# jh-jeong/ContraD

Hardware: AMD Instinct MI355X
Metric: discriminator-step images/sec (ContraD, SimCLR aug) (higher is better)
Workload: dtype f32; 1 GPU; SNDCGAN + ContraD D-step, CIFAR-10 32x32, global batch 512, simclr aug, nonsat loss, Adam(2e-4,(0.5,0.999)), random-init weights; global_batch=512, per_gpu_batch=512, parallelism=dp1, losses_finite=True, launch=hipGraph replay, rccl_ranks=1

## Files before the change

### contrad_amd/csrc/common.h

```cpp
#pragma once
#include <hip/hip_runtime.h>
#include <stdint.h>

#define CONTRAD_WAVE 64

#define CONTRAD_CHECK_LAUNCH()                       \
  do {                                               \
    hipError_t e__ = hipGetLastError();              \
    if (e__ != hipSuccess) return (int)e__;          \
  } while (0)

#define CONTRAD_ARG(cond)                            \
  do {                                               \
    if (!(cond)) return -22;            \
  } while (0)

#include <stdlib.h>
#ifdef CONTRAD_DEV_SWITCHES
static inline const char* contrad_dev_env(const char* name) { return getenv(name); }
#else
static inline const char* contrad_dev_env(const char*) { return nullptr; }
#endif
static inline bool contrad_dev_on(const char* name) { const char* e = contrad_dev_env(name); return !(e && e[0] == '0'); }
static inline bool contrad_dev_off_by_default(const char* name) { const char* e = contrad_dev_env(name); return e && e[0] == '1'; }
static inline int contrad_dev_int(const char* name, int dflt) { const char* e = contrad_dev_env(name); return e ? atoi(e) : dflt; }
static inline long long contrad_dev_ll(const char* name, long long dflt) { const char* e = contrad_dev_env(name); return e ? atoll(e) : dflt; }

typedef float f32x16 __attribute__((ext_vector_type(16)));
typedef float f32x4 __attribute__((ext_vector_type(4)));

static inline int cdiv(int a, int b) { return (a + b - 1) / b; }
__device__ __forceinline__ int cdiv_dev(int a, int b) { return (a + b - 1) / b; }
static inline long long cdivll(long long a, long long b) { return (a + b - 1) / b; }

__device__ __forceinline__ int xcd_remap(int b, int nb) {
  const int xcd = b & 7;
  const int q = nb >> 3, r = nb & 7;
  const int base = (xcd < r) ? xcd * (q + 1) : r * (q + 1) + (xcd - r) * q;
  return base + (b >> 3);
}

__device__ __forceinline__ float wave_sum(float v) {
#pragma unroll
  for (int o = 32; o > 0; o >>= 1) v += __shfl_xor(v, o, 64);
  return v;
}
__device__ __forceinline__ float wave_max(float v) {
#pragma unroll
  for (int o = 32; o > 0; o >>= 1) v = fmaxf(v, __shfl_xor(v, o, 64));
  return v;
}

__device__ __forceinline__ float block_sum(float v, float* red) {
  v = wave_sum(v);
  const int lane = threadIdx.x & 63, w = threadIdx.x >> 6, nw = (blockDim.x + 63) >> 6;
  __syncthreads();
  if (lane == 0) red[w] = v;
  __syncthreads();
  float t = 0.f;
  for (int i = 0; i < nw; ++i) t += red[i];
  return t;
}
```

### contrad_amd/csrc/conv_small.hip

```cpp
#include "common.h"
#include "../../include/contrad_hip.h"

namespace {

#ifndef RGB_MIN_WAVES
#define RGB_MIN_WAVES 3
#endif
typedef float f32x2 __attribute__((ext_vector_type(2)));
__device__ __forceinline__ f32x2 pk_fma(f32x2 a, f32x2 b, f32x2 c) { return __builtin_elementwise_fma(a, b, c); }

constexpr int MAX_TAPS = 9;
constexpr int MAX_CIN = 4;

struct RgbArgs {
  const float* img;
  const float* wp;
  const float* bias;
  float* y;
  int N, Cin, H, W, K, ldy, ldw, k, pad, TH;
  float in_scale, in_shift, slope, gain;
};

__device__ __forceinline__ void stage_halo(float* lds, const RgbArgs& a, int n, int h0) {
  const int HW = a.W + 2 * a.pad, HH = a.TH + 2 * a.pad;
// ... 186 lines not shown
  const long long total = (long long)a.N * a.H * a.W;
  for (long long pix0 = (long long)blockIdx.x * slots; pix0 < total; pix0 += (long long)gridDim.x * slots) {
    const long long pix = pix0 + slot;
    const bool live = pix < total;
    const long long pp = live ? pix : 0;
    const int wq = (int)(pp % a.W);
    const int h = (int)((pp / a.W) % a.H);
    const int n = (int)(pp / ((long long)a.W * a.H));
    float acc[MAX_CIN] = {0.f, 0.f, 0.f, 0.f};
    float4 md[CH];
#pragma unroll
    for (int q = 0; q < CH; ++q)
      md[q] = a.mod ? *reinterpret_cast<const float4*>(a.mod + (size_t)n * a.K + (q * tpp + cg) * 4)
                    : make_float4(1.f, 1.f, 1.f, 1.f);
#pragma unroll
    for (int kh = 0; kh < KSZ; ++kh) {
      const int ho = h + a.pad - kh;
#pragma unroll
      for (int kw = 0; kw < KSZ; ++kw) {
        const int wo = wq + a.pad - kw;
        const bool ok = live && (unsigned)ho < (unsigned)a.H && (unsigned)wo < (unsigned)a.W;
        const float m = ok ? 1.f : 0.f;
#pragma unroll
        for (int q = 0; q < CH; ++q) {
          const float4 g = *reinterpret_cast<const float4*>(
              a.gy + (ok ? ((size_t)(n * a.H + ho) * a.W + wo) * a.ldy + (q * tpp + cg) * 4 : 0));
#pragma unroll
          for (int c = 0; c < MAX_CIN; ++c) {
            const float4 ww = w[q][(kh * KSZ + kw) * MAX_CIN + c];
            acc[c] += m * (g.x * md[q].x * ww.x + g.y * md[q].y * ww.y + g.z * md[q].z * ww.z + g.w * md[q].w * ww.w);
          }
        }
      }
    }
#pragma unroll
    for (int c = 0; c < MAX_CIN; ++c)
      for (int o = tpp >> 1; o > 0; o >>= 1) acc[c] += __shfl_xor(acc[c], o, 64);
    if (live && cg < a.C) {
      float v = (cg == 0) ? acc[0] : (cg == 1) ? acc[1] : (cg == 2) ? acc[2] : acc[3];
      v += a.bias ? a.bias[cg] : 0.f;
      const size_t o = ((size_t)(n * a.C + cg) * a.H + h) * a.W + wq;
      if (a.residual) v += a.residual[o];
      if (a.act == 1) v = tanhf(v);
      a.out[o] = v * a.out_scale + a.out_shift;
    }
  }
}

constexpr int DG_CK = 32;
constexpr int DG_PS = DG_CK + 4;
__global__ __launch_bounds__(256) void rgb_dgrad3_tile_kernel(const float* __restrict__ gy, const float* __restrict__ wp,
                                                              const float* __restrict__ bias, float* __restrict__ out,
                                                              int N, int C, int H, int W, int K, int ldy, int ldw, int TH,
                                                              int act, float out_scale, float out_shift) {
  extern __shared__ __attribute__((aligned(16))) float tile[];
  const int tiles_h = cdiv_dev(H, TH);
  const int n = blockIdx.x / tiles_h, h0 = (blockIdx.x % tiles_h) * TH;
  const int HW2 = W + 2, HH2 = TH + 2;
  float* wl = tile + (size_t)HH2 * HW2 * DG_PS;
  const int r = threadIdx.x / W, c = threadIdx.x - r * W;
  const bool live = threadIdx.x < TH * W && h0 + r < H;
  float acc[3] = {0.f, 0.f, 0.f};
  for (int k0 = 0; k0 < K; k0 += DG_CK) {
    __syncthreads();
    for (int e = threadIdx.x; e < HH2 * HW2 * (DG_CK / 4); e += blockDim.x) {
      const int q = e % (DG_CK / 4), p = e / (DG_CK / 4);
      const int pr = p / HW2, pc = p - pr * HW2;
      const int h = h0 - 1 + pr, w = pc - 1;
      float4 v = make_float4(0.f, 0.f, 0.f, 0.f);
      if ((unsigned)h < (unsigned)H && (unsigned)w < (unsigned)W)
        v = *reinterpret_cast<const float4*>(gy + ((size_t)(n * H + h) * W + w) * ldy + k0 + q * 4);
      *reinterpret_cast<float4*>(tile + (size_t)p * DG_PS + q * 4) = v;
    }
    for (int e = threadIdx.x; e < 9 * 3 * (DG_CK / 4); e += blockDim.x) {
      const int q = e % (DG_CK / 4), tc = e / (DG_CK / 4);
      const int tap = tc / 3, cc = tc - tap * 3;
      float4 v = make_float4(0.f, 0.f, 0.f, 0.f);
      if (cc < C) v = *reinterpret_cast<const float4*>(wp + (size_t)(tap * C + cc) * ldw + k0 + q * 4);
      *reinterpret_cast<float4*>(wl + tc * DG_CK + q * 4) = v;
    }
    __syncthreads();
    if (live) {
#pragma unroll
      for (int kh = 0; kh < 3; ++kh)
#pragma unroll
        for (int kw = 0; kw < 3; ++kw) {
          const float4* g4 = reinterpret_cast<const float4*>(tile + (size_t)((r + 2 - kh) * HW2 + (c + 2 - kw)) * DG_PS);
          const float4* w4 = reinterpret_cast<const float4*>(wl + (kh * 3 + kw) * 3 * DG_CK);
#pragma unroll
          for (int q = 0; q < DG_CK / 4; ++q) {
            const float4 g = g4[q];
#pragma unroll
            for (int cc = 0; cc < 3; ++cc) {
              const float4 ww = w4[cc * (DG_CK / 4) + q];
              acc[cc] = fmaf(g.x, ww.x, fmaf(g.y, ww.y, fmaf(g.z, ww.z, fmaf(g.w, ww.w, acc[cc]))));
            }
          }
        }
    }
  }
  if (live) {
#pragma unroll
    for (int cc = 0; cc < 3; ++cc) {
      if (cc < C) {
        float v = acc[cc] + (bias ? bias[cc] : 0.f);
        if (act == 1) v = tanhf(v);
        out[((size_t)(n * C + cc) * H + h0 + r) * W + c] = v * out_scale + out_shift;
      }
    }
  }
}

int rgb_common_check(int N, int Cin, int H, int W, int K, int k, int ldy, int ldw) {
  CONTRAD_ARG(N > 0 && H > 0 && W > 0 && Cin == 3);
  CONTRAD_ARG(k == 1 || k == 3);
  CONTRAD_ARG(K >= 4 && (K & 3) == 0 && K <= 1024 && (1024 % K) == 0);
  CONTRAD_ARG(ldy >= K && (ldy & 3) == 0 && (ldw & 3) == 0 && ldw >= K);
  return 0;
}

int pick_th(int W) { int th = 1024 / W; return th < 1 ? 1 : (th > 32 ? 32 : th); }

}

extern "C" int contrad_rgb_conv_fwd(const float* img, const float* wp, const float* bias, float* y, int N,
                                    int Cin, int H, int W, int K, int k, int ldy, int ldw, float in_scale,
                                    float in_shift, float slope, float gain, contrad_stream_t stream) {
  int rc = rgb_common_check(N, Cin, H, W, K, k, ldy, ldw);
  if (rc) return rc;
  CONTRAD_ARG(img && wp && y);
  RgbArgs a{};
  a.img = img; a.wp = wp; a.bias = bias; a.y = y;
  a.N = N; a.Cin = Cin; a.H = H; a.W = W; a.K = K; a.ldy = ldy; a.ldw = ldw; a.k = k; a.pad = k / 2;
  a.TH = pick_th(W);
  a.in_scale = in_scale; a.in_shift = in_shift; a.slope = slope; a.gain = gain;
  const int tiles = N * cdiv(H, a.TH);
  const int grid = tiles < 4096 ? tiles : 4096;
  const size_t smem = (size_t)Cin * (a.TH + 2 * a.pad) * (W + 2 * a.pad) * sizeof(float);
  CONTRAD_ARG(smem <= 64 * 1024);
  if (k == 3) hipLaunchKernelGGL((rgb_conv_fwd_kernel<3, 3>), dim3(grid), dim3(256), smem, (hipStream_t)stream, a);
  else hipLaunchKernelGGL((rgb_conv_fwd_kernel<1, 3>), dim3(grid), dim3(256), smem, (hipStream_t)stream, a);
  CONTRAD_CHECK_LAUNCH();
  return 0;
}

static int rgb_wgrad_grid(int N, int H, int W, int k) {
  const int tiles = N * cdiv(H, pick_th(W));
  const int cap = (k == 3) ? 768 : 2048;
  return tiles < cap ? tiles : cap;
}

extern "C" long long contrad_rgb_conv_wgrad_workspace_bytes(int N, int Cin, int H, int W, int K, int k) {
  return (long long)rgb_wgrad_grid(N, H, W, k) * (k * k * Cin + 1) * K * (long long)sizeof(float);
}

extern "C" int contrad_rgb_conv_wgrad(const float* img, const float* gy, float* dwp, float* dbias, int N,
                                      int Cin, int H, int W, int K, int k, int ldy, int ldw, float in_scale,
                                      float in_shift, float* workspace, long long workspace_bytes,
                                      contrad_stream_t stream) {
  int rc = rgb_common_check(N, Cin, H, W, K, k, ldy, ldw);
  if (rc) return rc;
  CONTRAD_ARG(img && gy && dwp && workspace);
  CONTRAD_ARG(workspace_bytes >= contrad_rgb_conv_wgrad_workspace_bytes(N, Cin, H, W, K, k));
  RgbWgradArgs a{};
  a.img = img; a.gy = gy; a.partial = workspace;
  a.N = N; a.Cin = Cin; a.H = H; a.W = W; a.K = K; a.ldy = ldy; a.k = k; a.pad = k / 2; a.TH = pick_th(W);
  a.in_scale = in_scale; a.in_shift = in_shift;
  const int grid = rgb_wgrad_grid(N, H, W, k);
  size_t smem = (size_t)Cin * (a.TH + 2 * a.pad) * (W + 2 * a.pad) * sizeof(float);
  const size_t red = 256 * sizeof(float4);
  if (smem < red) smem = red;
  CONTRAD_ARG(smem <= 64 * 1024);
  if (k == 3) hipLaunchKernelGGL((rgb_conv_wgrad_kernel<3, 3>), dim3(grid), dim3(256), smem, (hipStream_t)stream, a);
  else hipLaunchKernelGGL((rgb_conv_wgrad_kernel<1, 3>), dim3(grid), dim3(256), smem, (hipStream_t)stream, a);
  CONTRAD_CHECK_LAUNCH();
  const int rows = k * k * Cin;
  hipLaunchKernelGGL(rgb_wgrad_reduce_kernel, dim3(cdiv((rows + 1) * K, 16)), dim3(256), 0,
                     (hipStream_t)stream, workspace, grid, rows, K, dwp, ldw, dbias);
  CONTRAD_CHECK_LAUNCH();
  return 0;
}

extern "C" int contrad_rgb_conv_dgrad(const float* gy, const float* wp, const float* bias, const float* mod,
                                      const float* residual, float* out, int N, int C, int H, int W, int K,
                                      int k, int ldy, int ldw, int act, float out_scale, float out_shift,
                                      contrad_stream_t stream) {
  CONTRAD_ARG(gy && wp && out && N > 0 && H > 0 && W > 0 && C >= 1 && C <= MAX_CIN);
  CONTRAD_ARG((k == 1 || k == 3) && K >= 16 && K <= 512 && (K & (K - 1)) == 0 && ldy >= K && (ldy & 3) == 0);
  CONTRAD_ARG(K <= 256 || k == 1);
  CONTRAD_ARG(ldw >= K && (ldw & 3) == 0 && (act == 0 || act == 1));
  RgbDgradArgs a{};
  a.gy = gy; a.wp = wp; a.bias = bias; a.out = out; a.mod = mod; a.residual = residual;
  a.N = N; a.C = C; a.H = H; a.W = W; a.K = K; a.ldy = ldy; a.ldw = ldw; a.k = k; a.pad = k / 2;
  a.act = act; a.out_scale = out_scale; a.out_shift = out_shift;
  const long long total = (long long)N * H * W;
  if (k == 3 && !mod && !residual && C <= 3 && (K % DG_CK) == 0 && W <= 256) {
    const int TH = 256 / W < 1 ? 1 : (256 / W > H ? H : 256 / W);
    const size_t smem = ((size_t)(TH + 2) * (W + 2) * DG_PS + 9 * 3 * DG_CK) * sizeof(float);
    if (smem <= 64 * 1024) {
      hipLaunchKernelGGL(rgb_dgrad3_tile_kernel, dim3(N * cdiv(H, TH)), dim3(256), smem, (hipStream_t)stream, gy, wp, bias,
                         out, N, C, H, W, K, ldy, ldw, TH, act, out_scale, out_shift);
      CONTRAD_CHECK_LAUNCH();
      return 0;
    }
  }
  const int ch = (K > 256) ? 2 : 1;
  const int slots = 256 / (K / (4 * ch));
  long long grid = (total + slots - 1) / slots;
  if (grid > 4096) grid = 4096;
  if (k == 3) hipLaunchKernelGGL((rgb_conv_dgrad_kernel<3, 1>), dim3((int)grid), dim3(256), 0, (hipStream_t)stream, a);
  else if (ch == 1) hipLaunchKernelGGL((rgb_conv_dgrad_kernel<1, 1>), dim3((int)grid), dim3(256), 0, (hipStream_t)stream, a);
  else hipLaunchKernelGGL((rgb_conv_dgrad_kernel<1, 2>), dim3((int)grid), dim3(256), 0, (hipStream_t)stream, a);
  CONTRAD_CHECK_LAUNCH();
  return 0;
}
```

### contrad_amd/csrc/elementwise.hip

```cpp
#include "common.h"
#include "../../include/contrad_hip.h"

namespace {

constexpr int COLS_PER_THREAD = 8;

template <bool SQ>
__global__ __launch_bounds__(256) void colstats_partial_kernel(const float* __restrict__ x, long long M, int K,
                                                               int ld, int rows_per_block,
                                                               float* __restrict__ partial) {
  __shared__ float red[4][64 * COLS_PER_THREAD + 1];
  __shared__ float red2[4][64 * COLS_PER_THREAD + 1];
  const int tx = threadIdx.x & 63, ty = threadIdx.x >> 6;
  const int cbase = blockIdx.y * 64 * COLS_PER_THREAD;
  const long long r0 = (long long)blockIdx.x * rows_per_block;
  const long long r1 = (r0 + rows_per_block < M) ? r0 + rows_per_block : M;
  float s[COLS_PER_THREAD], q[COLS_PER_THREAD];
#pragma unroll
  for (int j = 0; j < COLS_PER_THREAD; ++j) { s[j] = 0.f; q[j] = 0.f; }
  for (long long r = r0 + ty; r < r1; r += 4) {
    const float* row = x + r * ld;
#pragma unroll
    for (int j = 0; j < COLS_PER_THREAD; ++j) {
      const int c = cbase + tx + 64 * j;
// ... 53 lines not shown
  __syncthreads();
  const int nstat = SQ ? 2 : 1;
  if (rr == 0 && cok) {
    float4 t = red[0][cq];
    for (int g = 1; g < RPP; ++g) { const float4 u = red[g][cq]; t.x += u.x; t.y += u.y; t.z += u.z; t.w += u.w; }
    *reinterpret_cast<float4*>(partial + ((size_t)blockIdx.x * nstat + 0) * K + c) = t;
    if (SQ) {
      float4 t2 = red2[0][cq];
      for (int g = 1; g < RPP; ++g) { const float4 u = red2[g][cq]; t2.x += u.x; t2.y += u.y; t2.z += u.z; t2.w += u.w; }
      *reinterpret_cast<float4*>(partial + ((size_t)blockIdx.x * nstat + 1) * K + c) = t2;
    }
  }
}

constexpr int CSR_E = 16, CSR_P = 16;
__global__ __launch_bounds__(256) void colstats_reduce_kernel(const float* __restrict__ partial, int nblocks,
                                                              int nstat, int K, float* __restrict__ out,
                                                              int accumulate) {
  __shared__ float red[CSR_P][CSR_E + 1];
  const int ex = threadIdx.x % CSR_E, py = threadIdx.x / CSR_E;
  const int e = blockIdx.x * CSR_E + ex;
  const int E = nstat * K;
  float s0 = 0.f, s1 = 0.f, s2 = 0.f, s3 = 0.f;
  if (e < E) {
    int b = py;
    for (; b + 3 * CSR_P < nblocks; b += 4 * CSR_P) {
      s0 += partial[(size_t)b * E + e];
      s1 += partial[(size_t)(b + CSR_P) * E + e];
      s2 += partial[(size_t)(b + 2 * CSR_P) * E + e];
      s3 += partial[(size_t)(b + 3 * CSR_P) * E + e];
    }
    for (; b < nblocks; b += CSR_P) s0 += partial[(size_t)b * E + e];
  }
  red[py][ex] = (s0 + s1) + (s2 + s3);
  __syncthreads();
  if (py == 0 && e < E) {
    float s = 0.f;
#pragma unroll
    for (int r = 0; r < CSR_P; ++r) s += red[r][ex];
    out[e] = accumulate ? out[e] + s : s;
  }
}

__global__ void bn_relu_apply_kernel(const float* __restrict__ x, float* __restrict__ y, long long M, int K,
                                     int ldx, int ldy, const float* __restrict__ stats, float count,
                                     const float* __restrict__ gamma, const float* __restrict__ beta,
                                     float eps, int perm_hw) {
  const long long total = M * K;
  const float inv_n = 1.f / count;
  for (long long e = (long long)blockIdx.x * blockDim.x + threadIdx.x; e < total;
       e += (long long)gridDim.x * blockDim.x) {
    const long long r = e / K;
    const int c = (int)(e - r * K);
    const float mean = stats[c] * inv_n;
    const float var = fmaxf(stats[K + c] * inv_n - mean * mean, 0.f);
    const float v = (x[r * ldx + c] - mean) * rsqrtf(var + eps) * gamma[c] + beta[c];
    const float o = v > 0.f ? v : 0.f;
    if (perm_hw > 1) {
      const int ch = c / perm_hw, hw = c - ch * perm_hw;
      y[r * ldy + (size_t)hw * (K / perm_hw) + ch] = o;
    } else {
      y[r * ldy + c] = o;
    }
  }
}

__global__ __launch_bounds__(256) void bn_relu_bwd_stats_kernel(const float* __restrict__ dy,
                                                                const float* __restrict__ x, long long M, int K,
                                                                int ld, const float* __restrict__ stats, float count,
                                                                const float* __restrict__ gamma,
                                                                const float* __restrict__ beta, float eps,
                                                                int rows_per_block, float* __restrict__ partial) {
  __shared__ float red[4][64 * COLS_PER_THREAD + 1];
  __shared__ float red2[4][64 * COLS_PER_THREAD + 1];
  const int tx = threadIdx.x & 63, ty = threadIdx.x >> 6;
  const int cbase = blockIdx.y * 64 * COLS_PER_THREAD;
  const long long r0 = (long long)blockIdx.x * rows_per_block;
  const long long r1 = (r0 + rows_per_block < M) ? r0 + rows_per_block : M;
  float s[COLS_PER_THREAD], q[COLS_PER_THREAD], mu[COLS_PER_THREAD], rs[COLS_PER_THREAD], ga[COLS_PER_THREAD],
      be[COLS_PER_THREAD];
#pragma unroll
  for (int j = 0; j < COLS_PER_THREAD; ++j) {
    s[j] = 0.f; q[j] = 0.f;
    const int c = cbase + tx + 64 * j;
    if (c < K) {
      mu[j] = stats[c] / count;
      rs[j] = rsqrtf(fmaxf(stats[K + c] / count - mu[j] * mu[j], 0.f) + eps);
      ga[j] = gamma[c]; be[j] = beta[c];
    } else { mu[j] = 0.f; rs[j] = 0.f; ga[j] = 0.f; be[j] = 0.f; }
  }
  for (long long r = r0 + ty; r < r1; r += 4) {
#pragma unroll
    for (int j = 0; j < COLS_PER_THREAD; ++j) {
      const int c = cbase + tx + 64 * j;
      if (c < K) {
        const float xh = (x[r * ld + c] - mu[j]) * rs[j];
        const float g = (xh * ga[j] + be[j] > 0.f) ? dy[r * ld + c] : 0.f;
        s[j] += g;
        q[j] = fmaf(g, xh, q[j]);
      }
    }
  }
#pragma unroll
  for (int j = 0; j < COLS_PER_THREAD; ++j) { red[ty][tx + 64 * j] = s[j]; red2[ty][tx + 64 * j] = q[j]; }
  __syncthreads();
  for (int e = threadIdx.x; e < 64 * COLS_PER_THREAD; e += blockDim.x) {
    const int c = cbase + e;
    if (c < K) {
      partial[((size_t)blockIdx.x * 2 + 0) * K + c] = red[0][e] + red[1][e] + red[2][e] + red[3][e];
      partial[((size_t)blockIdx.x * 2 + 1) * K + c] = red2[0][e] + red2[1][e] + red2[2][e] + red2[3][e];
// ... 368 lines not shown
```

### contrad_amd/csrc/igemm.hip

```cpp
#include "common.h"
#include <stdlib.h>
#include <string.h>
#include <algorithm>
#include <utility>
#include "../../include/contrad_hip.h"

namespace {

enum { MODE_FWD = 0, MODE_DGRAD = 1, MODE_WGRAD = 2 };
#ifndef IGEMM_BK
#define IGEMM_BK 16
#endif
constexpr int BK = IGEMM_BK;
#ifndef IGEMM_MIN_WAVES
#define IGEMM_MIN_WAVES 4
#endif
constexpr int NTHREADS = 256;

struct IgemmArgs {
  const float* A;
  const float* B;
  float* C;
  const float* bias;
  const float* addend;
// ... 856 lines not shown
  if (g_plan_override.splits > 0) want = g_plan_override.splits;
  if (want < 1) want = 1;
  long long pps = cdivll(ptiles, want);
  if (pps < 4) pps = 4;
  if (pps > ptiles) pps = ptiles;
  p.tps = (int)pps;
  p.splits = (int)cdivll(ptiles, pps);
  if (d->K <= 32 && p.bm == 128 && vec_ok(d, MODE_WGRAD) && lean_ok(d, MODE_WGRAD, pps)) p.bn = 32;
  return p;
}

__global__ __launch_bounds__(256) void fwd_k1_kernel(const float* __restrict__ x, const float* __restrict__ w, long long M,
                                                     int C, int ldx, int ldw, const float* __restrict__ bias, float slope,
                                                     float gain, float* __restrict__ y, int ldy,
                                                     const float* __restrict__ addend) {
  const int lane = threadIdx.x & 63;
  const long long m = (long long)blockIdx.x * 4 + (threadIdx.x >> 6);
  if (m >= M) return;
  const float* xr = x + m * ldx;
  float acc = 0.f;
  for (int c = lane; c < C; c += 64) acc += xr[c] * w[(long long)c * ldw];
#pragma unroll
  for (int o = 32; o >= 1; o >>= 1) acc += __shfl_xor(acc, o, 64);
  if (lane == 0) {
    float v = acc + (bias ? bias[0] : 0.f);
    v = (v > 0.f) ? v : v * slope;
    v *= gain;
    if (addend) v += addend[m * ldy];
    y[m * ldy] = v;
  }
}

__global__ void fwd_reduce_kernel(const float* __restrict__ ws, int splits, long long M, int Ncol,
                                  const float* __restrict__ bias, float slope, float gain, float* __restrict__ y,
                                  int ldy, const float* __restrict__ addend) {
  const long long total = M * Ncol;
  for (long long e = (long long)blockIdx.x * blockDim.x + threadIdx.x; e < total;
       e += (long long)gridDim.x * blockDim.x) {
    float v = 0.f;
    for (int k = 0; k < splits; ++k) v += ws[(long long)k * total + e];
    const long long m = e / Ncol;
    const int c = (int)(e - m * Ncol);
    if (bias) v += bias[c];
    v = (v > 0.f) ? v : v * slope;
    v *= gain;
    if (addend) v += addend[m * ldy + c];
    y[m * ldy + c] = v;
  }
}

void split_plan(long long M, int Ncol, int t_total, double flops, FwdPlan* p) {
  static const int cand[4][2] = {{128, 128}, {64, 128}, {128, 64}, {64, 64}};
  static const double rate[4] = {135e12, 128e12, 128e12, 115e12};
  static const int sp[8] = {1, 2, 3, 4, 6, 8, 12, 16};
  if (g_plan_override.bm > 0) {
    const int s_ = std::max(1, g_plan_override.splits);
    p->bm = g_plan_override.bm; p->bn = g_plan_override.bn;
    p->tps = cdiv(t_total, s_);
    p->splits = cdiv(t_total, p->tps);
    return;
  }
  double best = 1e30;
  for (int i = (Ncol > 64 ? 0 : 2); i < 4; ++i)
    for (int j = 0; j < 8; ++j) {
      const int s_ = sp[j];
      const int tps = cdiv(t_total, s_);
      if (s_ > 1 && tps < 8) break;
      const int splits = cdiv(t_total, tps);
      const long long tm = cdivll(M, cand[i][0]), tn = cdivll(Ncol, cand[i][1]);
      const double blocks = (double)(tm * tn) * splits;
      const double waste = (double)(tm * cand[i][0]) * (double)(tn * cand[i][1]) / ((double)M * Ncol);
      const double fill = blocks >= 768.0 ? 1.0 : blocks / 768.0;
      double t = flops * waste / (rate[i] * fill);
      if (splits > 1) t += (2.0 * splits + 1.0) * (double)M * Ncol * 4.0 / 4e12 + 4e-6;
      if (t < best) { best = t; p->bm = cand[i][0]; p->bn = cand[i][1]; p->splits = splits; p->tps = tps; }
    }
}

bool fwd_k1_ok(const contrad_conv_desc* d) {
  return d->K == 1 && d->KH == 1 && d->KW == 1 && d->H == 1 && d->W == 1 && d->stride == 1 && d->pad == 0;
}

bool splitk_enabled() {
  static const bool on = contrad_dev_on("CONTRAD_IGEMM_SPLITK");
  return on;
}

constexpr double PIXMAJOR_MAX_VALID = 0.80;
constexpr double PIXMAJOR_WGRAD_MAX_VALID = 0.85;

bool pixmajor_enabled() {
  static const bool on = contrad_dev_on("CONTRAD_PIXMAJOR");
  return on;
}

double fwd_valid_tap_fraction(const contrad_conv_desc* d) {
  long long vh = 0, vw = 0;
  for (int ho = 0; ho < d->Ho; ++ho)
    for (int kh = 0; kh < d->KH; ++kh) vh += (unsigned)(ho * d->stride - d->pad + kh) < (unsigned)d->H;
  for (int wo = 0; wo < d->Wo; ++wo)
    for (int kw = 0; kw < d->KW; ++kw) vw += (unsigned)(wo * d->stride - d->pad + kw) < (unsigned)d->W;
  return (double)(vh * vw) / ((double)d->Ho * d->Wo * d->KH * d->KW);
}

constexpr double BORDER_MAX_VALID = 0.96;
bool border_classes_ok(const contrad_conv_desc* d, int mode, int bm);
bool fwd_pixmajor_ok(const contrad_conv_desc* d, int bm);
bool dgrad_pixmajor_ok(const contrad_conv_desc* d, int bm);
bool fwd_border_ok(const contrad_conv_desc* d, int bm, double valid) {
  return valid <= BORDER_MAX_VALID && !fwd_pixmajor_ok(d, bm) && border_classes_ok(d, MODE_FWD, bm);
}
bool dgrad_border_ok(const contrad_conv_desc* d, int bm, double valid) {
  return valid <= BORDER_MAX_VALID && !dgrad_pixmajor_ok(d, bm) && border_classes_ok(d, MODE_DGRAD, bm);
}

bool fwd_pixmajor_ok(const contrad_conv_desc* d, int bm) {
  if (!pixmajor_enabled() || d->Ho * d->Wo > 256 || d->N < bm) return false;
  if ((long long)bm * d->H * d->W * d->ldx * 4 >= (1ll << 30)) return false;
  if ((long long)bm * d->Ho * d->Wo * d->ldy * 4 >= (1ll << 31)) return false;
  return fwd_valid_tap_fraction(d) <= PIXMAJOR_MAX_VALID;
}

double dgrad_valid_tap_fraction(const contrad_conv_desc* d) {
  const int s = d->stride;
  long long valid = 0, all = 0;
  for (int h = 0; h < d->H; ++h) {
// ... 835 lines not shown
```

### contrad_amd/models/gan/sndcgan.py

```python
import contextlib

import torch
import torch.nn as nn
import torch.distributed as dist

from ... import ops
from ...hostio import upload
from ... import autograd_ops as A
from .base import BaseDiscriminator, SNParams, TinyHead, _Act, make_projection

_D_CONVS = [(3, 64, 3, 1, 1), (64, 128, 4, 2, 1), (128, 128, 3, 1, 1), (128, 256, 4, 2, 1),
            (256, 256, 3, 1, 1), (256, 512, 4, 2, 1), (512, 512, 3, 1, 1)]
_SLOPE = 0.1


def _flat_views(total_sizes, device):
    offs, tot = [], 0
    for n in total_sizes:
        offs.append(tot)
        tot += ops.round_up(n, 4)
    buf = torch.empty(max(tot, 4), device=device, dtype=torch.float32)
    return buf, [buf[o:o + n] for o, n in zip(offs, total_sizes)]


# ... 380 lines not shown
            layers.append(_WB((ci, co, k, k), co))
            if j < 3:
                layers += [BNParams(co), _Act(0.0)]
            else:
                layers.append(_Act(1.0))
        self.main = nn.Sequential(*layers)
        self.sync_bn = True
        self._packed = None
        self._packed_key = None
        self._packed_filters = {}

    def sample_latent(self, n_samples):
        _device = next(self.parameters()).device
        return upload(torch.empty(n_samples, self.nz).uniform_(-1, 1), _device)

    def invalidate_cache(self):
        self._packed, self._packed_key, self._packed_filters = None, None, {}

    def _weights(self):
        ws = [self.linear.weight] + [self.main[3 * j].weight for j in range(4)]
        key = tuple((w.data_ptr(), w._version) for w in ws)
        if self._packed_key != key:
            dev = ws[0].device
            specs = [ops.SnSpec(w, fixed_scale=1.0) for w in ws]
            sizes = [s.K * s.C * s.T for s in specs]
            buf, v = _flat_views(sizes, dev)
            wps = [v[i].view(s.T * s.C, s.K) for i, s in enumerate(specs)]
            ldws = [s.K for s in specs]
            offs, scr_n = ops.sn_scratch_floats(specs)
            scratch = torch.empty(scr_n, device=dev, dtype=torch.float32)
            sigma = torch.empty(len(specs), device=dev, dtype=torch.float32)
            ops.sn_weight_prep(specs, wps, ldws, False, scratch, offs, sigma)
            self._packed, self._packed_key, self._packed_buf = wps, key, buf
            self._packed_filters = {}
        return self._packed

    def _filters(self, N):
        if not ops.FILTER_PREP:
            return None
        pf = self._packed_filters.get(N)
        if pf is None:
            reqs, H, W = [], self.s_hb, self.s_wb
            for j in range(3):
                ci, co, k, s, p = self._CONVT[j]
                H, W = 2 * H, 2 * W
                reqs.append((1, ops.dgrad_desc((N, H, W, co), self._packed[1 + j], ci, k, k, s, p), self._packed[1 + j]))
            pf = self._packed_filters[N] = ops.filter_prep(reqs, self._packed[0].device)
        return pf

    def _bn(self, x2d, bn, conv_bias, out2d, perm_hw=1):
        if not self.training:
            mean = bn.running_mean if conv_bias is None else bn.running_mean - conv_bias
            stats = torch.stack([mean, bn.running_var + mean * mean]).contiguous()
            ops.bn_relu_apply(x2d, out2d, stats, 1.0, bn.weight, bn.bias, bn.eps, perm_hw)
            return
        count = float(x2d.shape[0])
        if ops.BN_FUSED and not _sync_on(self.sync_bn):
            stats = ops.bn_batch_stats(x2d, conv_bias, bn.momentum, bn.running_mean, bn.running_var, bn.num_batches_tracked)
            ops.bn_relu_apply(x2d, out2d, stats, count, bn.weight, bn.bias, bn.eps, perm_hw)
            return
        stats = ops.colstats(x2d, with_sq=True)
        if _sync_on(self.sync_bn):
            dist.all_reduce(stats)
            count *= dist.get_world_size()
        if self.training:
            ops.bn_running_update(stats, count, conv_bias, bn.momentum, bn.running_mean, bn.running_var,
                                  bn.num_batches_tracked)
        ops.bn_relu_apply(x2d, out2d, stats, count, bn.weight, bn.bias, bn.eps, perm_hw)

    def _forward_with_grad(self, z):
        N = z.shape[0]
        hb, wb = self.s_hb, self.s_wb
        f = 512 * hb * wb
        entries = [(f, self.nz, 1, 1.0, 0, 0)]
        groups = [(self.nz, f)]
        ws = [self.linear.weight]
        for j, (ci, co, k, s, p) in enumerate(self._CONVT):
            groups.append((k * k * co, ci))
            entries.append((ci, co, k * k, 1.0, j + 1, 0))
            ws.append(self.main[3 * j].weight)
        wp = A.PackWeightsFn.apply(A.PackMeta(entries, groups), *ws)
        z = z.contiguous().float()
        h0 = A.ConvBiasActFn.apply(z.view(N, 1, 1, self.nz), wp[0], self.linear.bias, (f, 1, 1, 1, 0), 1.0, 1.0)
        y0 = _BNReLUFn.apply(h0.view(N, f), self.norm_init.weight, self.norm_init.bias, self.norm_init, None,
                             self.sync_bn)
        x = y0.view(N, 512, hb, wb).permute(0, 2, 3, 1).contiguous()
        for j in range(3):
            ci, co, k, s, p = self._CONVT[j]
            H, W = x.shape[1], x.shape[2]
            y = A.ConvDgradFn.apply(x, wp[1 + j], (N, 2 * H, 2 * W, co), (ci, k, k, s, p))
            bn = self.main[3 * j + 1]
            y2 = _BNReLUFn.apply(y.view(-1, co), bn.weight, bn.bias, bn, self.main[3 * j].bias, self.sync_bn)
            x = y2.view(N, 2 * H, 2 * W, co)
        lin = A.RgbDgradFn.apply(x, wp[4], 3, (3, 1.0))
        return 0.5 * torch.tanh(lin + self.main[9].bias.view(1, 3, 1, 1)) + 0.5

    def forward(self, z):
        if not z.is_cuda:
            raise RuntimeError('contrad_amd.G_SNDCGAN runs on the MI355X HIP path only (no CPU fallback)')
        if torch.is_grad_enabled() and any(p.requires_grad for p in self.parameters()):
            if not self.training:
                raise NotImplementedError('eval-mode BatchNorm (running statistics) is not on the training path')
            return self._forward_with_grad(z)
        wps = self._weights()
        N = z.shape[0]
        filters = self._filters(N)
        hb, wb = self.s_hb, self.s_wb
        f = 512 * hb * wb
        z = z.contiguous().float()
        h0 = ops.conv2d_fwd(z.view(N, 1, 1, self.nz), wps[0], self.linear.bias, f, 1, 1, 1, 0).view(N, f)
        x = torch.empty((N, hb, wb, 512), device=z.device, dtype=torch.float32)
        self._bn(h0, self.norm_init, None, x.view(N, f), perm_hw=hb * wb)
        for j in range(3):
            ci, co, k, s, p = self._CONVT[j]
            H, W = x.shape[1], x.shape[2]
            y = ops.conv2d_dgrad(x, wps[1 + j], (N, 2 * H, 2 * W, co), k, k, s, p, filters=filters)
            y2 = ops.as_rows(y)
            self._bn(y2, self.main[3 * j + 1], self.main[3 * j].bias, y2)
            x = y
        return ops.rgb_conv_dgrad(x, wps[4], self.main[9].bias, 3, 3, act=1, out_scale=0.5, out_shift=0.5)
```

### contrad_amd/ops.py

```python
import ctypes
import math
import os

import torch

from ._lib import ConvDesc, ContrastProblem, FilterBatch, FilterJob, FILTER_MAX_JOBS, L2normProblem, lib


def _p(t):
    return ctypes.c_void_p(t.data_ptr()) if t is not None else ctypes.c_void_p(0)


_raw_stream = getattr(torch._C, '_cuda_getCurrentRawStream', None)


def _stream_handle():
    if _raw_stream is not None:
        return _raw_stream(torch.cuda.current_device())
    return torch.cuda.current_stream().cuda_stream


def _stream():
    return ctypes.c_void_p(_stream_handle())

# ... 453 lines not shown
        b.n = len(chunk)
        for j, s in enumerate(chunk):
            i = start + j
            L = b.layers[j]
            L.w = s.w.data_ptr()
            L.u = s.u.data_ptr() if s.u is not None else None
            L.v = s.v.data_ptr() if s.v is not None else None
            L.u_snap = u_snaps[i].data_ptr() if (u_snaps is not None and u_snaps[i] is not None) else None
            L.v_snap = v_snaps[i].data_ptr() if (v_snaps is not None and v_snaps[i] is not None) else None
            L.wp = wps[i].data_ptr()
            L.gwp = gwps[i].data_ptr() if gwps is not None else None
            L.gw = gws[i].data_ptr() if gws is not None else None
            L.K, L.C, L.T, L.ldw = s.K, s.C, s.T, ldws[i]
            L.fixed_scale = s.fixed_scale
            b.scratch_off[j] = offs[i]
        yield b, start


def sn_weight_prep(specs, wps, ldws, training, scratch, offs, sigma, u_snaps=None, v_snaps=None, eps=1e-12):
    for b, start in _sn_batches(specs, wps, ldws, offs, u_snaps, v_snaps):
        lib().call('contrad_sn_weight_prep', ctypes.byref(b), int(bool(training)), float(eps), _p(scratch),
                   ctypes.c_void_p(sigma.data_ptr() + 4 * start), _stream())


def sn_weight_grad(specs, wps, ldws, gwps, gws, scratch, offs, sigma, u_snaps=None, v_snaps=None):
    for b, start in _sn_batches(specs, wps, ldws, offs, u_snaps, v_snaps, gwps, gws):
        lib().call('contrad_sn_weight_grad', ctypes.byref(b), _p(scratch),
                   ctypes.c_void_p(sigma.data_ptr() + 4 * start), _stream())


def rgb_conv_fwd(img, wp, bias, K, k, in_scale, in_shift, slope, gain, out=None):
    _chk(img, 'img'); _chk(wp, 'wp'); _chk(bias, 'bias')
    if not img.is_contiguous():
        raise RuntimeError('contrad_hip: image batch must be contiguous NCHW')
    N, Cin, H, W = img.shape
    if out is None:
        out = torch.empty((N, H, W, K), device=img.device, dtype=torch.float32)
    lib().call('contrad_rgb_conv_fwd', _p(img), _p(wp), _p(bias), _p(out), N, Cin, H, W, K, k, _ld(out),
               wp.stride(0), float(in_scale), float(in_shift), float(slope), float(gain), _stream())
    return out


def rgb_conv_wgrad(img, gy, k, in_scale, in_shift, dwp, dbias=None):
    _chk(img, 'img'); _chk(gy, 'gy'); _chk(dwp, 'dwp')
    N, Cin, H, W = img.shape
    K = gy.shape[3]
    nbytes = lib().raw('contrad_rgb_conv_wgrad_workspace_bytes')(N, Cin, H, W, K, k)
    ws = _workspace(nbytes, img.device)
    lib().call('contrad_rgb_conv_wgrad', _p(img), _p(gy), _p(dwp), _p(dbias), N, Cin, H, W, K, k, _ld(gy),
               dwp.stride(0), float(in_scale), float(in_shift), _p(ws), ctypes.c_longlong(ws.numel() * 4), _stream())
    return dwp


def rgb_conv_dgrad(gy, wp, bias, C, k, act=0, out_scale=1.0, out_shift=0.0, out=None, mod=None, residual=None):
    _chk(gy, 'gy'); _chk(wp, 'wp'); _chk(bias, 'bias'); _chk(mod, 'mod'); _chk(residual, 'residual')
    N, H, W, K = gy.shape
    if out is None:
        out = torch.empty((N, C, H, W), device=gy.device, dtype=torch.float32)
    if mod is not None and (tuple(mod.shape) != (N, K) or not mod.is_contiguous()):
        raise RuntimeError('contrad_hip: mod must be a contiguous (N, K) tensor')
    if residual is not None and (tuple(residual.shape) != (N, C, H, W) or not residual.is_contiguous()):
        raise RuntimeError('contrad_hip: residual must be a contiguous (N, C, H, W) tensor')
    lib().call('contrad_rgb_conv_dgrad', _p(gy), _p(wp), _p(bias), _p(mod), _p(residual), _p(out), N, C, H, W, K, k,
               _ld(gy), wp.stride(0), int(act), float(out_scale), float(out_shift), _stream())
    return out


def colstats(x2d, with_sq=False, out=None, accumulate=False):
    _chk(x2d, 'x')
    M, K = x2d.shape
    ld = _ld(x2d)
    if out is None:
        out = torch.empty((2 if with_sq else 1, K), device=x2d.device, dtype=torch.float32)
    nbytes = lib().raw('contrad_colstats_workspace_bytes')(ctypes.c_longlong(M), K, int(with_sq))
    ws = _workspace(nbytes, x2d.device)
    lib().call('contrad_colstats', _p(x2d), ctypes.c_longlong(M), K, ld, int(with_sq), _p(out), int(accumulate),
               _p(ws), ctypes.c_longlong(ws.numel() * 4), _stream())
    return out


def as_rows(t):
    N, H, W, C = t.shape
    return t.as_strided((N * H * W, C), (_ld(t), 1), t.storage_offset())


def bn_relu_apply(x2d, y2d, stats, count, gamma, beta, eps=1e-5, perm_hw=1):
    M, K = x2d.shape
    lib().call('contrad_bn_relu_apply', _p(x2d), _p(y2d), ctypes.c_longlong(M), K, _ld(x2d), _ld(y2d), _p(stats),
               float(count), _p(gamma), _p(beta), float(eps), int(perm_hw), _stream())
    return y2d


def bn_running_update(stats, count, conv_bias, momentum, running_mean, running_var, num_batches_tracked=None):
    K = running_mean.numel()
    if num_batches_tracked is not None and (num_batches_tracked.dtype != torch.int64 or not num_batches_tracked.is_cuda):
        raise RuntimeError('contrad_hip: num_batches_tracked must be an int64 tensor on the device')
    lib().call('contrad_bn_running_update', _p(stats), float(count), K, _p(conv_bias), float(momentum),
               _p(running_mean), _p(running_var), _p(num_batches_tracked), _stream())


def bn_batch_stats(x2d, conv_bias, momentum, running_mean, running_var, num_batches_tracked=None):
    _chk(x2d, 'x')
    M, K = x2d.shape
    if num_batches_tracked is not None and (num_batches_tracked.dtype != torch.int64 or not num_batches_tracked.is_cuda):
        raise RuntimeError('contrad_hip: num_batches_tracked must be an int64 tensor on the device')
    out = torch.empty((2, K), device=x2d.device, dtype=torch.float32)
    nbytes = lib().raw('contrad_colstats_workspace_bytes')(ctypes.c_longlong(M), K, 1)
    ws = _workspace(nbytes, x2d.device)
    lib().call('contrad_bn_batch_stats', _p(x2d), ctypes.c_longlong(M), K, _ld(x2d), _p(out), _p(conv_bias),
               float(momentum), _p(running_mean), _p(running_var), _p(num_batches_tracked), _p(ws),
               ctypes.c_longlong(ws.numel() * 4), _stream())
# ... 885 lines not shown
```

### include/contrad_hip.h

```cpp
#ifndef CONTRAD_HIP_H
#define CONTRAD_HIP_H

#ifdef __cplusplus
extern "C" {
#endif

typedef void* contrad_stream_t;

int contrad_abi_version(void);

typedef struct {
  int N, H, W, C;
  int ldx;
  int Ho, Wo, K;
  int ldy;
  int KH, KW;
  int stride, pad;
  int ldw;
} contrad_conv_desc;

int contrad_conv2d_fwd(const contrad_conv_desc* d, const float* x, const float* wp, const float* bias,
                       float* y, float slope, float gain, float* workspace, long long workspace_bytes,
                       contrad_stream_t stream);
int contrad_conv2d_fwd_add(const contrad_conv_desc* d, const float* x, const float* wp, const float* bias,
// ... 80 lines not shown
} contrad_contrast_problem;
int contrad_contrast_fwd_batched(const contrad_contrast_problem* p, int n, contrad_stream_t stream);
int contrad_contrast_bwd_batched(const contrad_contrast_problem* p, int n, contrad_stream_t stream);
typedef struct {
  const float* u;
  float* z;
  float* inv_norm;
  const float* dz;
  float* du;
  int ldu, R, D;
  int accumulate;
  int zero_rows;
} contrad_l2norm_problem;
int contrad_l2norm_fwd_batched(const contrad_l2norm_problem* p, int n, float eps, contrad_stream_t stream);
int contrad_l2norm_bwd_batched(const contrad_l2norm_problem* p, int n, contrad_stream_t stream);

#define CONTRAD_SN_MAX_LAYERS 24
#define CONTRAD_SN_MAX_PARTIALS 256
typedef struct {
  const float* w;
  float* u;
  float* v;
  float* u_snap;
  float* v_snap;
  float* wp;
  const float* gwp;
  float* gw;
  int K, C, T, ldw;
  float fixed_scale;
} contrad_sn_layer;
typedef struct {
  int n;
  contrad_sn_layer layers[CONTRAD_SN_MAX_LAYERS];
  long long scratch_off[CONTRAD_SN_MAX_LAYERS];
} contrad_sn_batch;

long long contrad_sn_scratch_floats(int K, int C, int T);
int contrad_sn_weight_prep(const contrad_sn_batch* b, int training, float eps, float* scratch,
                           float* sigma_out, contrad_stream_t stream);
int contrad_sn_weight_grad(const contrad_sn_batch* b, float* scratch, const float* sigma,
                           contrad_stream_t stream);

int contrad_rgb_conv_fwd(const float* img, const float* wp, const float* bias, float* y, int N, int Cin,
                         int H, int W, int K, int k, int ldy, int ldw, float in_scale, float in_shift,
                         float slope, float gain, contrad_stream_t stream);
long long contrad_rgb_conv_wgrad_workspace_bytes(int N, int Cin, int H, int W, int K, int k);
int contrad_rgb_conv_wgrad(const float* img, const float* gy, float* dwp, float* dbias, int N, int Cin,
                           int H, int W, int K, int k, int ldy, int ldw, float in_scale, float in_shift,
                           float* workspace, long long workspace_bytes, contrad_stream_t stream);
int contrad_rgb_conv_dgrad(const float* gy, const float* wp, const float* bias, const float* mod,
                           const float* residual, float* out, int N, int C, int H, int W, int K, int k,
                           int ldy, int ldw, int act, float out_scale, float out_shift,
                           contrad_stream_t stream);

long long contrad_colstats_workspace_bytes(long long M, int K, int with_sq);
int contrad_colstats(const float* x, long long M, int K, int ld, int with_sq, float* out, int accumulate,
                     float* workspace, long long workspace_bytes, contrad_stream_t stream);
int contrad_bn_relu_apply(const float* x, float* y, long long M, int K, int ldx, int ldy, const float* stats,
                          float count, const float* gamma, const float* beta, float eps, int perm_hw,
                          contrad_stream_t stream);
int contrad_bn_relu_bwd_stats(const float* dy, const float* x, long long M, int K, int ld, const float* stats,
                              float count, const float* gamma, const float* beta, float eps, float* out2k,
                              float* workspace, long long workspace_bytes, contrad_stream_t stream);
int contrad_bn_relu_bwd_apply(const float* dy, const float* x, float* dx, long long M, int K, int ld,
                              const float* stats, float count, const float* gamma, const float* beta, float eps,
                              const float* bstats, contrad_stream_t stream);
int contrad_bn_running_update(const float* stats, float count, int K, const float* conv_bias, float momentum,
                              float* running_mean, float* running_var, long long* num_batches_tracked,
                              contrad_stream_t stream);
int contrad_bn_batch_stats(const float* x, long long M, int K, int ld, float* stats, const float* conv_bias,
                           float momentum, float* running_mean, float* running_var, long long* num_batches_tracked,
                           float* workspace, long long workspace_bytes, contrad_stream_t stream);
int contrad_gan_d_loss(const float* logits, int ld, int N, int kind, float* out3, float* grad,
                       contrad_stream_t stream);
int contrad_gan_g_loss(const float* logits, int ld, int N, int kind, float* out1, float* grad,
                       contrad_stream_t stream);

#define CONTRAD_ADAM_MAX_TENSORS 64
#define CONTRAD_ADAM_CHUNK 16384
typedef struct {
  float* p;
  const float* g;
  float* m;
  float* v;
  long long numel;
} contrad_adam_tensor;
typedef struct {
  int n;
  contrad_adam_tensor t[CONTRAD_ADAM_MAX_TENSORS];
  int block_start[CONTRAD_ADAM_MAX_TENSORS + 1];
} contrad_adam_batch;
int contrad_adam_step(const contrad_adam_batch* b, int step, float lr, float beta1, float beta2, float eps,
                      float grad_scale, contrad_stream_t stream);
int contrad_adam_step_dev(const contrad_adam_batch* b, const float* hyper_dev, float beta1, float beta2, float eps,
                          contrad_stream_t stream);
int contrad_axpby(float* y, const float* x, long long n, float a, float b, contrad_stream_t stream);
int contrad_pull_host(const float* host_pinned, float* dst, long long n, contrad_stream_t stream);

#define CONTRAD_AUG_NPARAM 16
long long contrad_simclr_workspace_bytes(int B, int H, int W);
int contrad_simclr_augment(const float* x, float* y, const float* params, int B, int H, int W,
                           int contrast_first, int has_contrast, float* workspace,
                           long long workspace_bytes, contrad_stream_t stream);
long long contrad_simclr_augment_bwd_workspace_bytes(int B, int H, int W);
int contrad_simclr_augment_bwd(const float* x, const float* params, const float* grad_out, float* grad_in,
                               int B, int H, int W, int contrast_first, int has_contrast, float* workspace,
// ... 148 lines not shown
```

Baseline: 48680 images/sec.

## Fuse last generator BatchNorm+ReLU into RGB dgrad tile load; refine split-K planner

When the generator runs without autograd, the final BatchNorm+ReLU is no longer written out as a separate activation. The RGB 3x3 dgrad tile kernel now computes per-channel BN coefficients and applies normalize+ReLU while staging the input into LDS. This removes one full read and write of the largest generator activation plus a kernel launch. Separately, the split-K GEMM planner now tries every split count from 1 to 16, models wave quantization over 768-block waves, and skips splits that leave a badly filled last wave. The planner change can pick different tilings for many GEMMs, so its effect may differ from layer to layer.

```diff
diff --git a/contrad_amd/csrc/common.h b/contrad_amd/csrc/common.h
--- a/contrad_amd/csrc/common.h
+++ b/contrad_amd/csrc/common.h
@@ -51,6 +51,24 @@
   return v;
 }
 
+struct BnCoef { float mean, rstd, gamma, beta; };
+__device__ __forceinline__ BnCoef bn_coef(const float* __restrict__ stats, int K, int c, float inv_n,
+                                          const float* __restrict__ gamma, const float* __restrict__ beta, float eps) {
+#pragma clang fp contract(off)
+  BnCoef k;
+  k.mean = stats[c] * inv_n;
+  const float var = fmaxf(fmaf(-k.mean, k.mean, stats[K + c] * inv_n), 0.f);
+  k.rstd = rsqrtf(var + eps);
+  k.gamma = gamma[c];
+  k.beta = beta[c];
+  return k;
+}
+__device__ __forceinline__ float bn_relu_value(float x, const BnCoef& k) {
+#pragma clang fp contract(off)
+  const float v = fmaf((x - k.mean) * k.rstd, k.gamma, k.beta);
+  return v > 0.f ? v : 0.f;
+}
+
 __device__ __forceinline__ float block_sum(float v, float* red) {
   v = wave_sum(v);
   const int lane = threadIdx.x & 63, w = threadIdx.x >> 6, nw = (blockDim.x + 63) >> 6;
diff --git a/contrad_amd/csrc/conv_small.hip b/contrad_amd/csrc/conv_small.hip
--- a/contrad_amd/csrc/conv_small.hip
+++ b/contrad_amd/csrc/conv_small.hip
@@ -262,7 +262,10 @@
 __global__ __launch_bounds__(256) void rgb_dgrad3_tile_kernel(const float* __restrict__ gy, const float* __restrict__ wp,
                                                               const float* __restrict__ bias, float* __restrict__ out,
                                                               int N, int C, int H, int W, int K, int ldy, int ldw, int TH,
-                                                              int act, float out_scale, float out_shift) {
+                                                              int act, float out_scale, float out_shift,
+                                                              const float* __restrict__ bn_stats, float bn_count,
+                                                              const float* __restrict__ bn_gamma,
+                                                              const float* __restrict__ bn_beta, float bn_eps) {
   extern __shared__ __attribute__((aligned(16))) float tile[];
   const int tiles_h = cdiv_dev(H, TH);
   const int n = blockIdx.x / tiles_h, h0 = (blockIdx.x % tiles_h) * TH;
@@ -273,14 +276,34 @@
   float acc[3] = {0.f, 0.f, 0.f};
   for (int k0 = 0; k0 < K; k0 += DG_CK) {
     __syncthreads();
-    for (int e = threadIdx.x; e < HH2 * HW2 * (DG_CK / 4); e += blockDim.x) {
-      const int q = e % (DG_CK / 4), p = e / (DG_CK / 4);
-      const int pr = p / HW2, pc = p - pr * HW2;
-      const int h = h0 - 1 + pr, w = pc - 1;
-      float4 v = make_float4(0.f, 0.f, 0.f, 0.f);
-      if ((unsigned)h < (unsigned)H && (unsigned)w < (unsigned)W)
-        v = *reinterpret_cast<const float4*>(gy + ((size_t)(n * H + h) * W + w) * ldy + k0 + q * 4);
-      *reinterpret_cast<float4*>(tile + (size_t)p * DG_PS + q * 4) = v;
+    if (bn_stats) {
+      const int q = threadIdx.x % (DG_CK / 4);
+      const float inv_n = 1.f / bn_count;
+      BnCoef co[4];
+#pragma unroll
+      for (int j = 0; j < 4; ++j) co[j] = bn_coef(bn_stats, K, k0 + q * 4 + j, inv_n, bn_gamma, bn_beta, bn_eps);
+      for (int e = threadIdx.x; e < HH2 * HW2 * (DG_CK / 4); e += 256) {
+        const int p = e / (DG_CK / 4);
+        const int pr = p / HW2, pc = p - pr * HW2;
+        const int h = h0 - 1 + pr, w = pc - 1;
+        float4 v = make_float4(0.f, 0.f, 0.f, 0.f);
+        if ((unsigned)h < (unsigned)H && (unsigned)w < (unsigned)W) {
+          v = *reinterpret_cast<const float4*>(gy + ((size_t)(n * H + h) * W + w) * ldy + k0 + q * 4);
+          v.x = bn_relu_value(v.x, co[0]); v.y = bn_relu_value(v.y, co[1]);
+          v.z = bn_relu_value(v.z, co[2]); v.w = bn_relu_value(v.w, co[3]);
+        }
+        *reinterpret_cast<float4*>(tile + (size_t)p * DG_PS + q * 4) = v;
+      }
+    } else {
+      for (int e = threadIdx.x; e < HH2 * HW2 * (DG_CK / 4); e += blockDim.x) {
+        const int q = e % (DG_CK / 4), p = e / (DG_CK / 4);
+        const int pr = p / HW2, pc = p - pr * HW2;
+        const int h = h0 - 1 + pr, w = pc - 1;
+        float4 v = make_float4(0.f, 0.f, 0.f, 0.f);
+        if ((unsigned)h < (unsigned)H && (unsigned)w < (unsigned)W)
+          v = *reinterpret_cast<const float4*>(gy + ((size_t)(n * H + h) * W + w) * ldy + k0 + q * 4);
+        *reinterpret_cast<float4*>(tile + (size_t)p * DG_PS + q * 4) = v;
+      }
     }
     for (int e = threadIdx.x; e < 9 * 3 * (DG_CK / 4); e += blockDim.x) {
       const int q = e % (DG_CK / 4), tc = e / (DG_CK / 4);
@@ -330,6 +353,23 @@
 }
 
 int pick_th(int W) { int th = 1024 / W; return th < 1 ? 1 : (th > 32 ? 32 : th); }
+
+int rgb_dgrad3_tile_launch(const float* gy, const float* wp, const float* bias, float* out, int N, int C, int H, int W,
+                           int K, int ldy, int ldw, int act, float out_scale, float out_shift, const float* bn_stats,
+                           float bn_count, const float* bn_gamma, const float* bn_beta, float bn_eps,
+                           contrad_stream_t stream, bool* launched) {
+  *launched = false;
+  if (!(C <= 3 && (K % DG_CK) == 0 && W <= 256)) return 0;
+  const int TH = 256 / W < 1 ? 1 : (256 / W > H ? H : 256 / W);
+  const size_t smem = ((size_t)(TH + 2) * (W + 2) * DG_PS + 9 * 3 * DG_CK) * sizeof(float);
+  if (smem > 64 * 1024) return 0;
+  *launched = true;
+  hipLaunchKernelGGL(rgb_dgrad3_tile_kernel, dim3(N * cdiv(H, TH)), dim3(256), smem, (hipStream_t)stream, gy, wp, bias,
+                     out, N, C, H, W, K, ldy, ldw, TH, act, out_scale, out_shift, bn_stats, bn_count, bn_gamma, bn_beta,
+                     bn_eps);
+  CONTRAD_CHECK_LAUNCH();
+  return 0;
+}
 
 }
 
@@ -404,15 +444,11 @@
   a.N = N; a.C = C; a.H = H; a.W = W; a.K = K; a.ldy = ldy; a.ldw = ldw; a.k = k; a.pad = k / 2;
   a.act = act; a.out_scale = out_scale; a.out_shift = out_shift;
   const long long total = (long long)N * H * W;
-  if (k == 3 && !mod && !residual && C <= 3 && (K % DG_CK) == 0 && W <= 256) {
-    const int TH = 256 / W < 1 ? 1 : (256 / W > H ? H : 256 / W);
-    const size_t smem = ((size_t)(TH + 2) * (W + 2) * DG_PS + 9 * 3 * DG_CK) * sizeof(float);
-    if (smem <= 64 * 1024) {
-      hipLaunchKernelGGL(rgb_dgrad3_tile_kernel, dim3(N * cdiv(H, TH)), dim3(256), smem, (hipStream_t)stream, gy, wp, bias,
-                         out, N, C, H, W, K, ldy, ldw, TH, act, out_scale, out_shift);
-      CONTRAD_CHECK_LAUNCH();
-      return 0;
-    }
+  if (k == 3 && !mod && !residual) {
+    bool launched;
+    const int rc = rgb_dgrad3_tile_launch(gy, wp, bias, out, N, C, H, W, K, ldy, ldw, act, out_scale, out_shift, nullptr,
+                                          1.f, nullptr, nullptr, 0.f, stream, &launched);
+    if (rc || launched) return rc;
   }
   const int ch = (K > 256) ? 2 : 1;
   const int slots = 256 / (K / (4 * ch));
@@ -424,3 +460,19 @@
   CONTRAD_CHECK_LAUNCH();
   return 0;
 }
+
+extern "C" int contrad_rgb_conv_dgrad_bn(const float* x, const float* stats, float count, const float* gamma,
+                                         const float* beta, float eps, const float* wp, const float* bias, float* out,
+                                         int N, int C, int H, int W, int K, int ldx, int ldw, int act, float out_scale,
+                                         float out_shift, contrad_stream_t stream) {
+  CONTRAD_ARG(x && wp && out && N > 0 && H > 0 && W > 0 && C >= 1 && C <= 3);
+  CONTRAD_ARG(stats ? (gamma && beta && count > 0.f) : (!gamma && !beta));
+  CONTRAD_ARG(K >= DG_CK && K <= 256 && (K & (K - 1)) == 0 && ldx >= K && (ldx & 3) == 0);
+  CONTRAD_ARG(ldw >= K && (ldw & 3) == 0 && (act == 0 || act == 1));
+  bool launched;
+  const int rc = rgb_dgrad3_tile_launch(x, wp, bias, out, N, C, H, W, K, ldx, ldw, act, out_scale, out_shift, stats, count,
+                                        gamma, beta, eps, stream, &launched);
+  if (rc) return rc;
+  CONTRAD_ARG(launched);
+  return 0;
+}
diff --git a/contrad_amd/csrc/elementwise.hip b/contrad_amd/csrc/elementwise.hip
--- a/contrad_amd/csrc/elementwise.hip
+++ b/contrad_amd/csrc/elementwise.hip
@@ -129,10 +129,7 @@
        e += (long long)gridDim.x * blockDim.x) {
     const long long r = e / K;
     const int c = (int)(e - r * K);
-    const float mean = stats[c] * inv_n;
-    const float var = fmaxf(stats[K + c] * inv_n - mean * mean, 0.f);
-    const float v = (x[r * ldx + c] - mean) * rsqrtf(var + eps) * gamma[c] + beta[c];
-    const float o = v > 0.f ? v : 0.f;
+    const float o = bn_relu_value(x[r * ldx + c], bn_coef(stats, K, c, inv_n, gamma, beta, eps));
     if (perm_hw > 1) {
       const int ch = c / perm_hw, hw = c - ch * perm_hw;
       y[r * ldy + (size_t)hw * (K / perm_hw) + ch] = o;
diff --git a/contrad_amd/csrc/igemm.hip b/contrad_amd/csrc/igemm.hip
--- a/contrad_amd/csrc/igemm.hip
+++ b/contrad_amd/csrc/igemm.hip
@@ -932,7 +932,6 @@
 void split_plan(long long M, int Ncol, int t_total, double flops, FwdPlan* p) {
   static const int cand[4][2] = {{128, 128}, {64, 128}, {128, 64}, {64, 64}};
   static const double rate[4] = {135e12, 128e12, 128e12, 115e12};
-  static const int sp[8] = {1, 2, 3, 4, 6, 8, 12, 16};
   if (g_plan_override.bm > 0) {
     const int s_ = std::max(1, g_plan_override.splits);
     p->bm = g_plan_override.bm; p->bn = g_plan_override.bn;
@@ -942,16 +941,18 @@
   }
   double best = 1e30;
   for (int i = (Ncol > 64 ? 0 : 2); i < 4; ++i)
-    for (int j = 0; j < 8; ++j) {
-      const int s_ = sp[j];
+    for (int s_ = 1; s_ <= 16; ++s_) {
       const int tps = cdiv(t_total, s_);
       if (s_ > 1 && tps < 8) break;
       const int splits = cdiv(t_total, tps);
       const long long tm = cdivll(M, cand[i][0]), tn = cdivll(Ncol, cand[i][1]);
-      const double blocks = (double)(tm * tn) * splits;
+      const long long blocks = tm * tn * splits;
       const double waste = (double)(tm * cand[i][0]) * (double)(tn * cand[i][1]) / ((double)M * Ncol);
-      const double fill = blocks >= 768.0 ? 1.0 : blocks / 768.0;
-      double t = flops * waste / (rate[i] * fill);
+      const double block_flops = flops * waste / (double)(tm * tn) * (double)tps / (double)t_total;
+      const long long full = blocks / 768, last = blocks % 768;
+      if (splits > 1 && full > 0 && last > 0 && last * 10 < 768 * 9) continue;
+      const double waves = full == 0 ? 1.0 : (double)full + (double)cdivll(last, 256) / 3.0;
+      double t = waves * 768.0 * block_flops / rate[i];
       if (splits > 1) t += (2.0 * splits + 1.0) * (double)M * Ncol * 4.0 / 4e12 + 4e-6;
       if (t < best) { best = t; p->bm = cand[i][0]; p->bn = cand[i][1]; p->splits = splits; p->tps = tps; }
     }
diff --git a/contrad_amd/models/gan/sndcgan.py b/contrad_amd/models/gan/sndcgan.py
--- a/contrad_amd/models/gan/sndcgan.py
+++ b/contrad_amd/models/gan/sndcgan.py
@@ -456,20 +456,21 @@
         if not self.training:
             mean = bn.running_mean if conv_bias is None else bn.running_mean - conv_bias
             stats = torch.stack([mean, bn.running_var + mean * mean]).contiguous()
-            ops.bn_relu_apply(x2d, out2d, stats, 1.0, bn.weight, bn.bias, bn.eps, perm_hw)
-            return
-        count = float(x2d.shape[0])
-        if ops.BN_FUSED and not _sync_on(self.sync_bn):
-            stats = ops.bn_batch_stats(x2d, conv_bias, bn.momentum, bn.running_mean, bn.running_var, bn.num_batches_tracked)
-            ops.bn_relu_apply(x2d, out2d, stats, count, bn.weight, bn.bias, bn.eps, perm_hw)
-            return
-        stats = ops.colstats(x2d, with_sq=True)
-        if _sync_on(self.sync_bn):
-            dist.all_reduce(stats)
-            count *= dist.get_world_size()
-        if self.training:
-            ops.bn_running_update(stats, count, conv_bias, bn.momentum, bn.running_mean, bn.running_var,
-                                  bn.num_batches_tracked)
+            count = 1.0
+        else:
+            count = float(x2d.shape[0])
+            if ops.BN_FUSED and not _sync_on(self.sync_bn):
+                stats = ops.bn_batch_stats(x2d, conv_bias, bn.momentum, bn.running_mean, bn.running_var,
+                                           bn.num_batches_tracked)
+            else:
+                stats = ops.colstats(x2d, with_sq=True)
+                if _sync_on(self.sync_bn):
+                    dist.all_reduce(stats)
+                    count *= dist.get_world_size()
+                ops.bn_running_update(stats, count, conv_bias, bn.momentum, bn.running_mean, bn.running_var,
+                                      bn.num_batches_tracked)
+        if out2d is None:
+            return stats, count, bn.weight, bn.bias, bn.eps
         ops.bn_relu_apply(x2d, out2d, stats, count, bn.weight, bn.bias, bn.eps, perm_hw)
 
     def _forward_with_grad(self, z):
@@ -520,6 +521,7 @@
             H, W = x.shape[1], x.shape[2]
             y = ops.conv2d_dgrad(x, wps[1 + j], (N, 2 * H, 2 * W, co), k, k, s, p, filters=filters)
             y2 = ops.as_rows(y)
-            self._bn(y2, self.main[3 * j + 1], self.main[3 * j].bias, y2)
+            fuse = j == 2 and not torch.is_grad_enabled() and 2 * W <= 256
+            bn_ops = self._bn(y2, self.main[3 * j + 1], self.main[3 * j].bias, None if fuse else y2)
             x = y
-        return ops.rgb_conv_dgrad(x, wps[4], self.main[9].bias, 3, 3, act=1, out_scale=0.5, out_shift=0.5)
+        return ops.rgb_conv_dgrad(x, wps[4], self.main[9].bias, 3, 3, act=1, out_scale=0.5, out_shift=0.5, bn=bn_ops)
diff --git a/contrad_amd/ops.py b/contrad_amd/ops.py
--- a/contrad_amd/ops.py
+++ b/contrad_amd/ops.py
@@ -529,11 +529,22 @@
     return dwp
 
 
-def rgb_conv_dgrad(gy, wp, bias, C, k, act=0, out_scale=1.0, out_shift=0.0, out=None, mod=None, residual=None):
+def rgb_conv_dgrad(gy, wp, bias, C, k, act=0, out_scale=1.0, out_shift=0.0, out=None, mod=None, residual=None, bn=None):
     _chk(gy, 'gy'); _chk(wp, 'wp'); _chk(bias, 'bias'); _chk(mod, 'mod'); _chk(residual, 'residual')
     N, H, W, K = gy.shape
     if out is None:
         out = torch.empty((N, C, H, W), device=gy.device, dtype=torch.float32)
+    if bn is not None:
+        stats, count, gamma, beta, eps = bn
+        if k != 3 or mod is not None or residual is not None:
+            raise RuntimeError('contrad_hip: BatchNorm operands go with the 3x3 kernel without mod / residual')
+        _chk(stats, 'stats'); _chk(gamma, 'gamma'); _chk(beta, 'beta')
+        if tuple(stats.shape) != (2, K) or not stats.is_contiguous() or gamma.numel() != K or beta.numel() != K:
+            raise RuntimeError('contrad_hip: stats must be a contiguous (2, K) tensor, gamma and beta K entries')
+        lib().call('contrad_rgb_conv_dgrad_bn', _p(gy), _p(stats), float(count), _p(gamma), _p(beta), float(eps), _p(wp),
+                   _p(bias), _p(out), N, C, H, W, K, _ld(gy), wp.stride(0), int(act), float(out_scale), float(out_shift),
+                   _stream())
+        return out
     if mod is not None and (tuple(mod.shape) != (N, K) or not mod.is_contiguous()):
         raise RuntimeError('contrad_hip: mod must be a contiguous (N, K) tensor')
     if residual is not None and (tuple(residual.shape) != (N, C, H, W) or not residual.is_contiguous()):
diff --git a/include/contrad_hip.h b/include/contrad_hip.h
--- a/include/contrad_hip.h
+++ b/include/contrad_hip.h
@@ -156,6 +156,10 @@
                            const float* residual, float* out, int N, int C, int H, int W, int K, int k,
                            int ldy, int ldw, int act, float out_scale, float out_shift,
                            contrad_stream_t stream);
+int contrad_rgb_conv_dgrad_bn(const float* x, const float* stats, float count, const float* gamma, const float* beta,
+                              float eps, const float* wp, const float* bias, float* out, int N, int C, int H, int W,
+                              int K, int ldx, int ldw, int act, float out_scale, float out_shift,
+                              contrad_stream_t stream);
 
 long long contrad_colstats_workspace_bytes(long long M, int K, int with_sq);
 int contrad_colstats(const float* x, long long M, int K, int ld, int with_sq, float* out, int accumulate,
```

After: 49020 images/sec, median of 6. Within noise of the previous version (+0.7%).
